# timlawrenz/DINO-X

Hardware: AMD Instinct MI355X
Metric: training images/sec (source samples; 2 global views each) ViT-S/16 224px bs256/GPU (higher is better)
Workload: dtype bf16; 1 GPU; ViT-S/16 224x224x3 2.5D slice stacks, scale-aware, 2 views/sample, DINO+Gram loss, AdamW+EMA; per_gpu_batch=256, global_batch=256, local_crops=0, out_dim=8192, parallelism=dp1, hipgraph=False

## Files before the change

### dino-x_amd/csrc/kernels.h

```cpp
#pragma once
#include <type_traits>

#include "gemm_common.h"
#include "knobs.h"

namespace dinox {

#define GEMM_VARIANTS(X)                                                                                                       \
  X(NtPp, "gemm_bf16_nt_pp") X(NtPp128, "gemm_bf16_nt_pp128") X(NtPp384, "gemm_bf16_nt_pp384") X(NtAreg, "gemm_bf16_nt_areg") \
  X(NtGlds, "gemm_bf16_nt_glds") X(Nt, "gemm_bf16_nt") X(TnBig, "gemm_bf16_tn_big") X(TnDma, "gemm_bf16_tn_dma") X(Tn, "gemm_bf16_tn")
#define X(member, name) member,
enum class GemmVariant { None, GEMM_VARIANTS(X) };
#undef X
#define X(member, name) name,
inline const char* gemm_variant_name(GemmVariant v) {
  static const char* const names[] = {nullptr, GEMM_VARIANTS(X)};
  return names[(int)v];
}
#undef X

int launch_gemm_f32(const GemmParams& p, hipStream_t st);
GemmVariant gemm_bf16_variant(const GemmParams& p);
int launch_gemm_bf16(const GemmParams& p, hipStream_t st);
int64_t gemm_bf16_ws_bytes(const GemmParams& p);
bool gemm_bf16_nt_glds_ok(const GemmParams& p);
int launch_gemm_bf16_nt_glds(const GemmParams& p, hipStream_t st);
bool gemm_bf16_nt_areg_ok(const GemmParams& p);
int launch_gemm_bf16_nt_areg(const GemmParams& p, hipStream_t st);
bool gemm_bf16_nt_pp_ok(const GemmParams& p);
int launch_gemm_bf16_nt_pp(const GemmParams& p, hipStream_t st);
bool gemm_bf16_nt_pp128_ok(const GemmParams& p);
int launch_gemm_bf16_nt_pp128(const GemmParams& p, hipStream_t st);
bool gemm_bf16_nt_pp384_ok(const GemmParams& p);
int launch_gemm_bf16_nt_pp384(const GemmParams& p, hipStream_t st);
bool gemm_bf16_nt_pp384_ln_ok(int64_t M, int K);
int launch_gemm_bf16_nt_pp384_ln(const void* a, const void* w, const float* bias, const float* residual, float* x_out, const float* gamma,
                                 const float* beta, float eps, void* y, float* mean, float* rstd, int64_t M, int K, hipStream_t st);
int pp384_lnbwd_tiles(int64_t M);
int launch_gemm_bf16_nt_pp384_lnbwd(const void* a, const void* w, const float* x, const float* gamma, const float* mean, const float* rstd,
                                    float* dx, const float* dx_add, void* dx_lowp, float* ws, int64_t M, int K, hipStream_t st);
int tn_big_plan(const GemmParams& p, int& tiles_m, int& tiles_n, int& splits, int64_t& kps);
int64_t tn_big_ws_bytes(const GemmParams& p);
int launch_gemm_bf16_tn_big(const GemmParams& p, hipStream_t st, int& splits_out, int& tiles_n_out);

int launch_attention_ref_fwd(const void* qkv, void* o, float* lse, int B, int N, int heads, int d, int dtype, hipStream_t st);
int launch_attention_ref_bwd(const void* d_o, const void* qkv, const void* o, const float* lse, void* dqkv, int B, int N, int heads, int d, int dtype, hipStream_t st);
int launch_attention_bf16_fwd(const void* qkv, void* o, float* lse, int B, int N, int heads, int d, hipStream_t st);
int launch_attention_bf16_bwd(const void* d_o, const void* qkv, const void* o, const float* lse, void* dqkv, float* ws, int B, int N, int heads, int d, hipStream_t st);
bool attention_qkv_fused_ok(int B, int N, int heads, int d, int D);
int launch_attention_qkv_fused_fwd(const void* x, const void* w, const float* bias, void* o, void* qkv_out, float* lse, int B, int N, int heads, int d, int D, hipStream_t st);
int launch_attention_flash_fwd(const void* qkv, void* o, float* lse, int B, int N, int heads, int d, hipStream_t st);
int launch_attention_flash_bwd(const void* d_o, const void* qkv, const void* o, const float* lse, void* dqkv, float* ws, int B, int N, int heads, int d, hipStream_t st);

enum { EPI_ACT_PLAIN = 0, EPI_ACT_GELU = 1, EPI_ACT_DGELU = 2 };

template <typename F>
static inline int with_epilogue_case(const GemmParams& p, F&& f) {
  const int act = (p.epilogue & DINOX_EPI_GELU) ? EPI_ACT_GELU : (p.epilogue & DINOX_EPI_DGELU) ? EPI_ACT_DGELU : EPI_ACT_PLAIN;
  const bool res = (p.epilogue & DINOX_EPI_RESIDUAL) != 0;
  auto cases = [&](auto out) -> int {
    switch (act * 2 + (res ? 1 : 0)) {
      case 0: return f(out, std::integral_constant<int, EPI_ACT_PLAIN>{}, std::false_type{});
      case 1: return f(out, std::integral_constant<int, EPI_ACT_PLAIN>{}, std::true_type{});
      case 2: return f(out, std::integral_constant<int, EPI_ACT_GELU>{}, std::false_type{});
      case 4: return f(out, std::integral_constant<int, EPI_ACT_DGELU>{}, std::false_type{});
      default: return DINOX_EUNSUPPORTED;
    }
  };
  return p.out_dtype == DINOX_BF16 ? cases(std::integral_constant<int, DINOX_BF16>{}) : cases(std::integral_constant<int, DINOX_F32>{});
}

struct PersistPlan {
  int tiles_n, units, order, stagger;
  unsigned grid;
};
static inline bool persist_plan(const GemmParams& p, int bm, int bn, int stagger_auto, PersistPlan& pl) {
  const int64_t tiles_n = ceil_div(p.N, (int64_t)bn), units = ceil_div(p.M, (int64_t)bm) * tiles_n;
  if (units > 0x3fffffff) return false;
  const int64_t ncu = device_cu_count();
  pl = {(int)tiles_n, (int)units, knob_int("DINOX_PP_ORDER", 1), knob_int("DINOX_PP_STAGGER", stagger_auto), (unsigned)(units < ncu ? units : ncu)};
  return true;
}

}
```

### dino-x_amd/csrc/loss.hip

```cpp
#include "common.h"

namespace dinox {

constexpr int CE_THREADS = 256;

__global__ __launch_bounds__(CE_THREADS) void dino_ce_kernel(const float* __restrict__ s, const float* __restrict__ t,
                                                             const float* __restrict__ center, float inv_ts, float inv_tt,
                                                             float gscale, float* __restrict__ ds,
                                                             float* __restrict__ row_loss, int rows, int K) {
  __shared__ float red[16];
  const int i = blockIdx.x, B = rows / 2;
  const int pi = (i + B) % rows;
  const float* sr = s + (int64_t)i * K;
  const float* tr = t + (int64_t)pi * K;
  float ms = -INFINITY, mt = -INFINITY;
  for (int k = threadIdx.x; k < K; k += CE_THREADS) {
    ms = fmaxf(ms, sr[k] * inv_ts);
    mt = fmaxf(mt, (tr[k] - center[k]) * inv_tt);
  }
  ms = block_max(ms, red);
  mt = block_max(mt, red);
  float ss = 0.f, st = 0.f;
  for (int k = threadIdx.x; k < K; k += CE_THREADS) {
    ss += expf(sr[k] * inv_ts - ms);
    st += expf((tr[k] - center[k]) * inv_tt - mt);
  }
  ss = block_sum(ss, red);
  st = block_sum(st, red);
  const float log_ss = logf(ss), inv_ss = 1.0f / ss, inv_st = 1.0f / st;
  float acc = 0.f;
  for (int k = threadIdx.x; k < K; k += CE_THREADS) {
    const float zs = sr[k] * inv_ts - ms;
    const float tp = expf((tr[k] - center[k]) * inv_tt - mt) * inv_st;
    acc -= tp * (zs - log_ss);
    if (ds) ds[(int64_t)i * K + k] = gscale * (expf(zs) * inv_ss - tp) * inv_ts / (float)rows;
  }
  acc = block_sum(acc, red);
  if (threadIdx.x == 0) row_loss[i] = acc;
}

__global__ __launch_bounds__(CE_THREADS) void dino_teacher_stats_kernel(const float* __restrict__ t, const float* __restrict__ center,
                                                                        float inv_tt, float* __restrict__ tmax, float* __restrict__ tinv, int K) {
  __shared__ float red[16];
  const int i = blockIdx.x;
  const float* tr = t + (int64_t)i * K;
  float m = -INFINITY;
  for (int k = threadIdx.x; k < K; k += CE_THREADS) m = fmaxf(m, (tr[k] - center[k]) * inv_tt);
  m = block_max(m, red);
  float a = 0.f;
  for (int k = threadIdx.x; k < K; k += CE_THREADS) a += expf((tr[k] - center[k]) * inv_tt - m);
  a = block_sum(a, red);
  if (threadIdx.x == 0) {
    tmax[i] = m;
// ... 188 lines not shown
}

extern "C" int dinox_colmean(const float* t, float* out, int rows, int K, void* stream) {
  DX_REQUIRE(t && out && rows > 0 && K > 0, DINOX_EINVAL, "colmean: bad arguments");
  if (K % 4 == 0 && (((uintptr_t)t | (uintptr_t)out) & 15) == 0)
    hipLaunchKernelGGL(colmean_kernel, dim3((unsigned)ceil_div(K / 4, 64)), dim3(256), 0, as_stream(stream), t, out, rows, K);
  else
    hipLaunchKernelGGL(colmean_scalar_kernel, dim3((unsigned)ceil_div(K, 256)), dim3(256), 0, as_stream(stream), t, out, rows, K);
  return check_launch("colmean");
}

extern "C" int dinox_center_ema(float* center, const float* batch_mean, float momentum, int K, void* stream) {
  DX_REQUIRE(center && batch_mean && K > 0, DINOX_EINVAL, "center_ema: bad arguments");
  hipLaunchKernelGGL(center_ema_kernel, dim3((unsigned)ceil_div(K, 256)), dim3(256), 0, as_stream(stream), center, batch_mean, momentum, K);
  return check_launch("center_ema");
}

extern "C" int dinox_gram_normalize(const float* sfeats, const float* tfeats, void* cat, void* catneg, void* shat,
                                    float* snorm, int V, int N, int D, int out_dtype, void* stream) {
  DX_REQUIRE(sfeats && tfeats && cat && catneg && shat && snorm, DINOX_EINVAL, "gram_normalize: null pointer");
  DX_REQUIRE(V > 0 && N > 1 && D > 0, DINOX_EINVAL, "gram_normalize: V=%d N=%d D=%d", V, N, D);
  DX_REQUIRE(out_dtype == DINOX_F32 || out_dtype == DINOX_BF16, DINOX_EINVAL, "gram_normalize: dtype %d", out_dtype);
  const unsigned blocks = (unsigned)ceil_div((int64_t)V * (N - 1), 4);
  if (out_dtype == DINOX_F32)
    hipLaunchKernelGGL((gram_normalize_kernel<DINOX_F32>), dim3(blocks), dim3(256), 0, as_stream(stream), sfeats, tfeats, cat, catneg, shat, snorm, V, N, D);
  else
    hipLaunchKernelGGL((gram_normalize_kernel<DINOX_BF16>), dim3(blocks), dim3(256), 0, as_stream(stream), sfeats, tfeats, cat, catneg, shat, snorm, V, N, D);
  return check_launch("gram_normalize");
}

extern "C" int dinox_sqsum(const float* x, int64_t n, float scale, float* loss, float* ws, void* stream) {
  DX_REQUIRE(x && loss && ws && n > 0, DINOX_EINVAL, "sqsum: bad arguments");
  int64_t blocks = ceil_div(n, 256 * 8);
  if (blocks > 1024) blocks = 1024;
  hipStream_t st = as_stream(stream);
  hipLaunchKernelGGL(sqsum_partial_kernel, dim3((unsigned)blocks), dim3(256), 0, st, x, n, ws);
  hipLaunchKernelGGL(final_sum_kernel, dim3(1), dim3(256), 0, st, ws, (int)blocks, scale, loss);
  return check_launch("sqsum");
}

extern "C" int dinox_gram_normalize_bwd(const float* dxh, const void* shat, const float* snorm, const float* sfeats,
                                        float* dfeats, int V, int N, int D, int shat_dtype, int accumulate, void* stream) {
  (void)sfeats;
  DX_REQUIRE(dxh && shat && snorm && dfeats, DINOX_EINVAL, "gram_normalize_bwd: null pointer");
  DX_REQUIRE(V > 0 && N > 1 && D > 0, DINOX_EINVAL, "gram_normalize_bwd: V=%d N=%d D=%d", V, N, D);
  DX_REQUIRE(shat_dtype == DINOX_F32 || shat_dtype == DINOX_BF16, DINOX_EINVAL, "gram_normalize_bwd: dtype %d", shat_dtype);
  const unsigned blocks = (unsigned)ceil_div((int64_t)V * (N - 1), 4);
  if (shat_dtype == DINOX_F32)
    hipLaunchKernelGGL((gram_normalize_bwd_kernel<DINOX_F32>), dim3(blocks), dim3(256), 0, as_stream(stream), dxh, shat, snorm, dfeats, V, N, D, accumulate);
  else
    hipLaunchKernelGGL((gram_normalize_bwd_kernel<DINOX_BF16>), dim3(blocks), dim3(256), 0, as_stream(stream), dxh, shat, snorm, dfeats, V, N, D, accumulate);
  return check_launch("gram_normalize_bwd");
}
```

### dino-x_amd/dinox/_lib.py

```python
from __future__ import annotations

import ctypes as C
import os

import torch

_HERE = os.path.dirname(os.path.abspath(__file__))
LIB_PATH = os.environ.get("DINOX_LIB") or os.path.join(_HERE, "libdinox_hip.so")

F32, BF16 = 0, 1
EPI_BIAS, EPI_GELU, EPI_DGELU, EPI_RESIDUAL, EPI_ACCUM, EPI_AUXGRAD = 1, 2, 4, 8, 16, 32

vp, i32, i64, f32 = C.c_void_p, C.c_int32, C.c_int64, C.c_float


class GemmArgs(C.Structure):
    _fields_ = [
        ("A", vp), ("B", vp), ("C", vp),
        ("M", i64), ("N", i64), ("K", i64),
        ("lda", i64), ("ldb", i64), ("ldc", i64),
        ("batch", i64), ("strideA", i64), ("strideB", i64), ("strideC", i64),
        ("transA", i32), ("transB", i32), ("in_dtype", i32), ("out_dtype", i32), ("epilogue", i32),
        ("alpha", f32),
        ("bias", vp), ("residual", vp), ("ldr", i64), ("aux", vp), ("ldaux", i64), ("colsum", vp), ("ws", vp),
# ... 9 lines not shown
        ("n1w", vp), ("n1b", vp), ("n2w", vp), ("n2b", vp), ("wqkv", vp), ("wproj", vp), ("w1", vp), ("w2", vp),
        ("bqkv", vp), ("bproj", vp), ("b1", vp), ("b2", vp),
    ]


class BlockBwdArgs(C.Structure):
    _fields_ = [
        ("V", i64), ("N", i64), ("D", i32), ("H", i32), ("heads", i32), ("reserved", i32),
        ("g", vp), ("g_lowp", vp), ("g_lowp_buf", vp),
        ("x0", vp), ("x1", vp), ("xn1", vp), ("xn2", vp), ("qkv", vp), ("o", vp), ("lse", vp), ("pre", vp), ("act", vp),
        ("mean1", vp), ("rstd1", vp), ("mean2", vp), ("rstd2", vp), ("n1w", vp), ("n2w", vp),
        ("wqkv_t", vp), ("wproj_t", vp), ("w1_t", vp), ("w2_t", vp),
        ("dwqkv", vp), ("dbqkv", vp), ("dwproj", vp), ("dbproj", vp), ("dw1", vp), ("db1", vp), ("dw2", vp), ("db2", vp),
        ("dn1w", vp), ("dn1b", vp), ("dn2w", vp), ("dn2b", vp),
        ("dpre", vp), ("dxn2", vp), ("d_o", vp), ("dqkv", vp), ("dxn1", vp), ("g1", vp), ("g1_lowp", vp), ("g0_lowp", vp),
        ("attn_ws", vp), ("ln_ws", vp), ("tn_ws", vp), ("tn_ws_bytes", i64),
    ]


SIGNATURES = {
    "dinox_version": (i32, []),
    "dinox_last_error": (C.c_char_p, []),
    "dinox_device_ok": (i32, []),
    "dinox_gemm": (i32, [C.POINTER(GemmArgs), vp]),
    "dinox_gemm_kernel_name": (C.c_char_p, [C.POINTER(GemmArgs)]),
    "dinox_gemm_ws_bytes": (i64, [C.POINTER(GemmArgs)]),
    "dinox_colsum": (i32, [vp, vp, i64, i64, i64, i32, i32, vp]),
    "dinox_linear_residual_ln_ok": (i32, [i64, i32, i32]),
    "dinox_linear_residual_ln": (i32, [vp, vp, vp, vp, vp, vp, vp, f32, vp, i32, vp, vp, i64, i32, i32, vp]),
    "dinox_layernorm_fwd": (i32, [vp, vp, vp, vp, vp, vp, i64, i32, f32, i32, vp]),
    "dinox_layernorm_bwd_ws_bytes": (i64, [i64, i32]),
    "dinox_layernorm_bwd": (i32, [vp, vp, vp, vp, vp, vp, vp, vp, vp, vp, vp, i64, i32, i32, i32, vp]),
    "dinox_linear_ln_bwd_ok": (i32, [i64, i32, i32]),
    "dinox_linear_ln_bwd": (i32, [vp, vp, vp, vp, vp, vp, vp, vp, vp, vp, vp, vp, i64, i32, i32, i32, vp]),
    "dinox_attention_fwd": (i32, [vp, vp, vp, i32, i32, i32, i32, i32, vp]),
    "dinox_attention_bwd_ws_bytes": (i64, [i32, i32, i32]),
    "dinox_attention_bwd": (i32, [vp, vp, vp, vp, vp, vp, i32, i32, i32, i32, i32, vp]),
    "dinox_qkv_attention_ok": (i32, [i32, i32, i32, i32, i32]),
    "dinox_qkv_attention_fwd": (i32, [vp, vp, vp, vp, vp, vp, i32, i32, i32, i32, i32, vp]),
    "dinox_patch_unfold": (i32, [vp, vp, i32, i32, i32, i32, i32, vp]),
    "dinox_patch_unfold_ld": (i32, [vp, vp, i32, i32, i32, i32, i32, i32, vp]),
    "dinox_tokens_fwd": (i32, [vp, vp, vp, vp, vp, vp, i32, i32, i32, i32, i32, vp]),
    "dinox_tokens_bwd": (i32, [vp, vp, vp, vp, vp, vp, i32, i32, i32, i32, i32, vp]),
    "dinox_scale_embed_fwd": (i32, [vp] * 12 + [i32, i32, i32, f32, vp]),
    "dinox_scale_embed_bwd_ws_bytes": (i64, [i32, i32, i32]),
    "dinox_scale_embed_bwd": (i32, [vp] * 17 + [i32, i32, i32, vp]),
    "dinox_dino_ce": (i32, [vp, vp, vp, f32, f32, f32, vp, vp, vp, i32, i32, vp]),
    "dinox_dino_ce_multi": (i32, [vp, vp, vp, f32, f32, f32, vp, vp, vp, i32, i32, i32, i32, vp]),
    "dinox_colmean": (i32, [vp, vp, i32, i32, vp]),
    "dinox_center_ema": (i32, [vp, vp, f32, i32, vp]),
    "dinox_gram_normalize": (i32, [vp, vp, vp, vp, vp, vp, i32, i32, i32, i32, vp]),
    "dinox_sqsum": (i32, [vp, i64, f32, vp, vp, vp]),
    "dinox_gram_normalize_bwd": (i32, [vp, vp, vp, vp, vp, i32, i32, i32, i32, i32, vp]),
    "dinox_slice_views_lds_bytes": (i64, [i32, i32]),
    "dinox_slice_views": (i32, [vp, vp, vp, vp, i32, i32, i32, vp]),
    "dinox_slice_views_patches": (i32, [vp, vp, vp, vp, i32, i32, i32, i32, i32, i32, vp]),
    "dinox_softmax_rows": (i32, [vp, vp, i64, i32, i32, i64, vp]),
    "dinox_softmax_bwd_rows": (i32, [vp, vp, vp, f32, i64, i32, i32, i64, vp]),
    "dinox_koleo_normalize": (i32, [vp, vp, vp, vp, i64, i32, f32, vp]),
    "dinox_koleo_nn": (i32, [vp, i64, vp, vp, i32, i32, i32, i32, vp, vp, vp]),
    "dinox_koleo_loss": (i32, [vp, i32, f32, vp, vp]),
    "dinox_koleo_bwd": (i32, [vp, vp, vp, vp, i32, i32, i32, i32, f32, f32, f32, vp, vp]),
    "dinox_adamw_ema": (i32, [vp, vp, vp, vp, vp, i64, f32, f32, f32, f32, f32, i32, f32, f32, vp, vp, vp]),
    "dinox_adamw_ema_dev": (i32, [vp, vp, vp, vp, vp, i64, vp, f32, f32, f32, f32, f32, f32, vp, vp, vp]),
    "dinox_sumsq": (i32, [vp, i64, vp, vp, vp]),
    "dinox_cast_bf16": (i32, [vp, vp, i64, vp]),
    "dinox_cast_transpose_bf16": (i32, [vp, vp, i32, i32, vp]),
    "dinox_cast_transpose_bf16_multi": (i32, [vp, vp, vp, i32, i64, vp]),
    "dinox_take_rows": (i32, [vp, vp, i64, i64, i32, i64, i32, vp]),
    "dinox_put_rows": (i32, [vp, vp, i64, i64, i32, i64, i32, i32, vp]),
    "dinox_axpy": (i32, [vp, vp, f32, i64, vp]),
    "dinox_lincomb3": (i32, [vp, vp, vp, f32, f32, vp, vp]),
    "dinox_zero": (i32, [vp, i64, vp]),
    "dinox_gelu_fwd": (i32, [vp, vp, i64, vp]),
    "dinox_gelu_bwd": (i32, [vp, vp, vp, i64, vp]),
    "dinox_block_forward": (i32, [C.POINTER(BlockFwdArgs), vp]),
    "dinox_block_backward": (i32, [C.POINTER(BlockBwdArgs), vp]),
    "dinox_retrieval_ws_bytes": (i64, [i64, i64, i64]),
    "dinox_retrieval_rank": (i32, [vp, i64, vp, i64, vp, i64, i64, i64, vp, vp, vp, vp, vp, vp]),
    "dinox_knn_ws_bytes": (i64, [i64, i64, i64, i32]),
    "dinox_knn_topk": (i32, [vp, i64, vp, i64, vp, i64, i64, i64, i32, vp, vp, vp, vp]),
    "dinox_gemm_timer_start": (i32, [i32]),
    "dinox_gemm_timer_stop": (i64, [C.c_char_p, i64]),
}


class DinoxLibraryError(ImportError):
    pass


def _load() -> C.CDLL:
    if not os.path.exists(LIB_PATH):
        raise DinoxLibraryError(
            f"{LIB_PATH} not found: the HIP kernel library is the only compute path of this package "
            "(no CPU/eager fallback). Build it with `python -c 'import __graft_entry__ as g; g.build()'` "
            "or `make -C dino-x_amd/csrc`.")
    try:
        lib = C.CDLL(LIB_PATH)
    except OSError as e:
        raise DinoxLibraryError(f"cannot load {LIB_PATH}: {e}") from e
    for name, (res, args) in SIGNATURES.items():
        try:
            fn = getattr(lib, name)
        except AttributeError as e:
            raise DinoxLibraryError(f"{LIB_PATH} does not export {name}; rebuild it") from e
        fn.restype = res
# ... 15 lines not shown
```

### dino-x_amd/dinox/engine.py

```python
from __future__ import annotations

import os
from dataclasses import dataclass
from typing import List, Optional, Tuple

import torch
import torch.distributed as dist

from . import ops
from .dp import GradBucketer, exchanging
from .schedule import get_lr


@dataclass
class StepHyperParams:
    lr: float = 1e-4
    min_lr: float = 1e-6
    warmup_steps: int = 2500
    max_steps: Optional[int] = None
    weight_decay: float = 0.04
    ema: float = 0.996
    teacher_temp: float = 0.04
    student_temp: float = 0.1
    center_momentum: float = 0.9
# ... 180 lines not shown
        dt = self.compute_dtype
        l0, l2 = head[0], head[2]
        pre0 = torch.empty((cls_op.shape[0], l0.weight.shape[0]), dtype=dt, device=cls_op.device) if train else None
        h0 = ops.gemm(cls_op, ops.weight_operand(l0.weight, dt), bias=l0.bias, gelu=True, aux=pre0, auxgrad=True, out_dtype=dt)
        out = ops.gemm(h0, ops.weight_operand(l2.weight, dt), bias=l2.bias, out_dtype=torch.float32)
        if train:
            ops.grad_sink.use(l0.weight, l0.bias, l2.weight, l2.bias)
        return out, (cls_op, h0, pre0)

    def _head_backward(self, head, saved, ds: torch.Tensor) -> torch.Tensor:
        dt = self.compute_dtype
        l0, l2 = head[0], head[2]
        cls_op, h0, pre0 = saved
        dy = ops.to_mode(ds, dt)
        if dt == torch.float32:
            dpre = ops.gemm(dy, l2.weight.detach(), transB=True, dgelu=True, aux=pre0, auxgrad=True, out_dtype=dt)
        else:
            dpre = ops.gemm(dy, ops.weight_operand(l2.weight, dt, transposed=True), dgelu=True, aux=pre0, auxgrad=True, out_dtype=dt)
        g2 = ops.weight_grad(dy, h0, l2.weight, l2.bias, True)
        if dt == torch.float32:
            dcls = ops.gemm(dpre, l0.weight.detach(), transB=True, out_dtype=dt)
        else:
            dcls = ops.gemm(dpre, ops.weight_operand(l0.weight, dt, transposed=True), out_dtype=dt)
        g0 = ops.weight_grad(dpre, cls_op, l0.weight, l0.bias, True)
        assert g2 == (None, None) and g0 == (None, None), "the head's parameters must live in the engine's gradient arena"
        return dcls

    def _losses_and_backward(self, s_feats, t_feats, batch, local_batch, local_spacing):
        hp, dt = self.hp, self.compute_dtype
        scale = 1.0 / self.accum
        V = s_feats.shape[0]
        with torch.no_grad():
            sf = s_feats.detach()
            t_out, _ = self._head_forward(self.teacher.head, ops.take_rows(t_feats, 0, dt), train=False)
            if local_batch is None:
                l_feats = None
                cls = ops.take_rows(sf, 0, dt)
            else:
                with torch.enable_grad():
                    l_feats = self.student.backbone(local_batch, spacing=local_spacing)
                lf = l_feats.detach()
                cls = ops.take_rows(sf, 0, dt, out_rows=V + lf.shape[0])
                ops.take_rows(lf, 0, dt, out=cls, out_row0=V)
            s_all, saved = self._head_forward(self.student.head, cls, train=True)
            if local_batch is None:
                l_dino, ds = ops.dino_ce(s_all, t_out, self.center, hp.student_temp, hp.teacher_temp, True, grad_scale=scale)
            else:
                l_dino, ds = ops.dino_ce_multi(s_all, t_out, self.center, hp.student_temp, hp.teacher_temp, 2, grad_scale=scale)
            bm = ops.colmean(t_out)
            bm_work = dist.all_reduce(bm, op=dist.ReduceOp.SUM, group=self.group, async_op=True) if exchanging(self.group) else None
            kstate = ops.koleo_begin(s_all[:V], group=self.group) if hp.koleo_weight > 0.0 else None
            dfeats = torch.empty_like(sf)
            l_gram = None
            if hp.gram_weight != 0.0:
                l_gram, gsaved = ops.gram_loss_fwd(sf, t_feats, dt)
                ops.gram_loss_bwd(gsaved, tuple(sf.shape), hp.gram_weight * scale, dfeats=dfeats, accumulate=False)
            else:
                ops.zero_(dfeats)
            l_koleo = None
            if kstate is not None:
                l_koleo, ksaved = ops.koleo_end(kstate)
                ops.axpy_(ds[:V], ops.koleo_bwd(ksaved, hp.koleo_weight * scale), 1.0)
            dcls = self._head_backward(self.student.head, saved, ds)
            ops.put_rows_(dfeats, 0, dcls)
            roots, grads = [s_feats], [dfeats]
            if l_feats is not None:
                dl = torch.empty_like(lf)
                ops.zero_(dl)
                ops.put_rows_(dl, 0, dcls, src_row0=V)
                roots.append(l_feats)
                grads.append(dl)
            loss = ops.lincomb3(l_dino, l_gram, l_koleo, hp.gram_weight, hp.koleo_weight)
        self._mark("loss")
        torch.autograd.backward(roots, grads)
        z = self._zero1
        return loss.reshape(()), l_dino.reshape(()), (l_gram if l_gram is not None else z).reshape(()), \
            (l_koleo if l_koleo is not None else z).reshape(()), bm, bm_work

    def _losses_and_backward_autograd(self, s_feats, t_feats, t_out, batch, local_batch, local_spacing):
        hp = self.hp
        if local_batch is None:
            s_out = self.student.head(s_feats[:, 0])
            l_dino = ops.DinoCEFn.apply(s_out, t_out, self.center, hp.student_temp, hp.teacher_temp)
        else:
            l_feats = self.student.backbone(local_batch, spacing=local_spacing)
            s_all = self.student.head(torch.cat([s_feats[:, 0], l_feats[:, 0]], 0))
            s_out = s_all[:s_feats.shape[0]]
            l_dino = ops.DinoCEMultiFn.apply(s_all, t_out, self.center, hp.student_temp, hp.teacher_temp, 2)
        bm = ops.colmean(t_out)
        bm_work = dist.all_reduce(bm, op=dist.ReduceOp.SUM, group=self.group, async_op=True) if exchanging(self.group) else None
        if hp.gram_weight != 0.0:
            l_gram = ops.GramLossFn.apply(s_feats, t_feats)
            loss = l_dino + hp.gram_weight * l_gram
        else:
            l_gram = torch.zeros((), device=batch.device)
            loss = l_dino
        if hp.koleo_weight > 0.0:
            l_koleo = ops.koleo_loss(s_out, group=self.group)
            loss = loss + hp.koleo_weight * l_koleo
        else:
            l_koleo = torch.zeros((), device=batch.device)
        self._mark("loss")
        (loss if self.accum == 1 else loss / self.accum).backward()
        return loss.detach(), l_dino.detach(), l_gram.detach(), l_koleo.detach(), bm, bm_work

    def scalars(self) -> dict:
        r = self.last
# ... 3 lines not shown
```

### dino-x_amd/dinox/ops.py

```python
from __future__ import annotations

import contextlib
import ctypes as C
import math
import operator
import os
import weakref
from typing import Optional

import torch

from . import _lib
from ._lib import BF16, EPI_ACCUM, EPI_AUXGRAD, EPI_BIAS, EPI_DGELU, EPI_GELU, EPI_RESIDUAL, F32, BlockBwdArgs, BlockFwdArgs, GemmArgs, check, lib

Tensor = torch.Tensor
_OVERRIDE: list = []


@contextlib.contextmanager
def compute_dtype(dtype: torch.dtype):
    if dtype not in (torch.float32, torch.bfloat16):
        raise ValueError("compute dtype must be torch.float32 or torch.bfloat16")
    _OVERRIDE.append(dtype)
    try:
# ... 1451 lines not shown
    assert src.dtype == torch.float32 and src.is_contiguous() and src.dim() == 3
    V, N, D = src.shape
    if out is None:
        out = torch.empty((out_rows or V, D), dtype=dt, device=src.device)
    check(lib.dinox_take_rows(src.data_ptr() + 4 * row * D, _p(out), V, N * D, D, out_row0, _code(dt), _stream()), "dinox_take_rows")
    return out


def put_rows_(dst: Tensor, row: int, src: Tensor, src_row0: int = 0, accumulate: bool = False) -> None:
    assert dst.dtype == torch.float32 and dst.is_contiguous() and dst.dim() == 3 and src.is_contiguous()
    V, N, D = dst.shape
    check(lib.dinox_put_rows(_p(src), dst.data_ptr() + 4 * row * D, V, N * D, D, src_row0, _code(src.dtype), int(accumulate), _stream()),
          "dinox_put_rows")


def axpy_(y: Tensor, x: Tensor, alpha: float) -> None:
    assert y.dtype == torch.float32 and x.dtype == torch.float32 and y.is_contiguous() and x.is_contiguous() and y.numel() == x.numel()
    check(lib.dinox_axpy(_p(y), _p(x), alpha, y.numel(), _stream()), "dinox_axpy")


def lincomb3(a: Tensor, b: Optional[Tensor], c: Optional[Tensor], wb: float, wc: float) -> Tensor:
    out = torch.empty(1, dtype=torch.float32, device=a.device)
    check(lib.dinox_lincomb3(_p(a), _p(b), _p(c), wb, wc, _p(out), _stream()), "dinox_lincomb3")
    return out


def zero_(t: Tensor) -> None:
    assert t.is_contiguous()
    check(lib.dinox_zero(_p(t), t.numel() * t.element_size(), _stream()), "dinox_zero")


def colmean(t: Tensor) -> Tensor:
    t = _c(t.float())
    out = torch.empty(t.shape[1], dtype=torch.float32, device=t.device)
    check(lib.dinox_colmean(_p(t), _p(out), t.shape[0], t.shape[1], _stream()), "dinox_colmean")
    return out


def center_ema_(center: Tensor, batch_mean: Tensor, momentum: float) -> None:
    assert center.is_contiguous() and center.dtype == torch.float32
    check(lib.dinox_center_ema(_p(center), _p(batch_mean), momentum, center.numel(), _stream()), "dinox_center_ema")


def gram_loss_fwd(sf: Tensor, tf: Tensor, dt: torch.dtype):
    _need_cuda(sf, tf)
    sf, tf = _c(sf.float()), _c(tf.float())
    V, N, D = sf.shape
    T = N - 1
    dev = sf.device
    cat = torch.empty((V, T, 2 * D), dtype=dt, device=dev)
    catneg = torch.empty((V, T, 2 * D), dtype=dt, device=dev)
    shat = torch.empty((V, T, D), dtype=dt, device=dev)
    snorm = torch.empty((V, T), dtype=torch.float32, device=dev)
    check(lib.dinox_gram_normalize(_p(sf), _p(tf), _p(cat), _p(catneg), _p(shat), _p(snorm), V, N, D, _code(dt), _stream()), "dinox_gram_normalize")
    diff = gemm(cat, catneg, out_dtype=torch.float32)
    loss = torch.empty(1, dtype=torch.float32, device=dev)
    ws = torch.empty(1024, dtype=torch.float32, device=dev)
    check(lib.dinox_sqsum(_p(diff), diff.numel(), 1.0 / float(V * T * T), _p(loss), _p(ws), _stream()), "dinox_sqsum")
    return loss, (diff, shat, snorm)


def gram_loss_bwd(saved, sf_shape, scale: float, dfeats: Optional[Tensor] = None, accumulate=False) -> Tensor:
    diff, shat, snorm = saved
    V, N, D = sf_shape
    T = N - 1
    dt = shat.dtype
    d_in = diff if dt == torch.float32 else cast_bf16(diff)
    dxh = gemm(d_in, shat, transA=True, transB=True, out_dtype=torch.float32, alpha=4.0 * scale / float(V * T * T))
    if dfeats is None:
        dfeats = torch.zeros((V, N, D), dtype=torch.float32, device=diff.device)
    check(lib.dinox_gram_normalize_bwd(_p(dxh), _p(shat), _p(snorm), None, _p(dfeats), V, N, D, _code(dt), int(accumulate), _stream()),
          "dinox_gram_normalize_bwd")
    return dfeats


class GramLossFn(torch.autograd.Function):

    @staticmethod
    def forward(ctx, sf, tf):
        dt = current_dtype()
        loss, saved = gram_loss_fwd(sf, tf, dt)
        ctx.save_for_backward(*saved)
        ctx.shape = tuple(sf.shape)
        return loss.reshape(())

    @staticmethod
    def backward(ctx, g):
        d = gram_loss_bwd(ctx.saved_tensors, ctx.shape, 1.0)
        return d * g, None


def koleo_begin(x: Tensor, group=None):
    import torch.distributed as dist
    _need_cuda(x)
    x = _c(x.float())
    V, D = x.shape
    dev = x.device
    from .dp import exchanging
    gather = exchanging(group)
    world = dist.get_world_size(group) if gather else 1
    rank = dist.get_rank(group) if gather else 0
    f = lambda *sh: torch.empty(sh, dtype=torch.float32, device=dev)
    xh, norm, sq = f(V, D), f(V), f(V)
    check(lib.dinox_koleo_normalize(_p(x), _p(xh), _p(norm), _p(sq), V, D, 1e-12, _stream()), "dinox_koleo_normalize")
    works = []
    if gather:
        xh_all, sq_all = f(world * V, D), f(world * V)
        works.append(dist.all_gather_into_tensor(xh_all, xh, group=group, async_op=True))
        works.append(dist.all_gather_into_tensor(sq_all, sq, group=group, async_op=True))
    else:
        xh_all, sq_all = xh, sq
    return (xh, xh_all, sq_all, norm, works, group, gather, world, rank, V, D)


def koleo_end(state, eps: float = 1e-8):
    import torch.distributed as dist
    xh, xh_all, sq_all, norm, works, group, gather, world, rank, V, D = state
    for w in works:
        w.wait()
    dev = xh.device
    f = lambda *sh: torch.empty(sh, dtype=torch.float32, device=dev)
    Vg, row0 = world * V, rank * V
    G = gemm_nt_f32_splitk(xh, xh_all)
    idx = torch.empty(V, dtype=torch.int32, device=dev)
    dmin = f(V)
    check(lib.dinox_koleo_nn(_p(G), Vg, _p(sq_all), _p(xh_all), row0, V, Vg, D, _p(idx), _p(dmin), _stream()), "dinox_koleo_nn")
# ... 186 lines not shown
```

### include/dinox.h

```cpp
#ifndef DINOX_H
#define DINOX_H

#include <stdint.h>

#ifdef __cplusplus
extern "C" {
#endif

#define DINOX_ABI_VERSION 3

#define DINOX_F32 0
#define DINOX_BF16 1

#define DINOX_OK 0
#define DINOX_EINVAL (-1)
#define DINOX_EUNSUPPORTED (-2)
#define DINOX_EALIGN (-3)

int dinox_version(void);
const char* dinox_last_error(void);
int dinox_device_ok(void);

#define DINOX_EPI_BIAS 1
#define DINOX_EPI_GELU 2
// ... 38 lines not shown
int dinox_layernorm_fwd(const float* x, const float* w, const float* b, void* y, float* mean, float* rstd,
                        int64_t rows, int dim, float eps, int out_dtype, void* stream);
int64_t dinox_layernorm_bwd_ws_bytes(int64_t rows, int dim);
int dinox_layernorm_bwd(const void* dy, const float* x, const float* w, const float* mean, const float* rstd,
                        float* dx, const float* dx_add, void* dx_lowp, float* dw, float* db, void* ws,
                        int64_t rows, int dim, int dy_dtype, int accumulate, void* stream);
int dinox_linear_ln_bwd_ok(int64_t M, int N, int K);
int dinox_linear_ln_bwd(const void* a, const void* w, const float* x, const float* gamma, const float* mean, const float* rstd,
                        float* dx, const float* dx_add, void* dx_lowp, float* dgamma, float* dbeta, void* ws, int64_t M, int N,
                        int K, int accumulate, void* stream);

int dinox_attention_fwd(const void* qkv, void* o, float* lse, int B, int N, int heads, int d, int dtype,
                        void* stream);
int dinox_softmax_rows(float* s, float* lse, int64_t rows, int n, int rows_per_image, int64_t lse_image_stride, void* stream);
int dinox_softmax_bwd_rows(float* s, float* dp, const float* lse, float scale, int64_t rows, int n, int rows_per_image,
                           int64_t lse_image_stride, void* stream);
int64_t dinox_attention_bwd_ws_bytes(int B, int N, int heads);
int dinox_attention_bwd(const void* d_o, const void* qkv, const void* o, const float* lse, void* dqkv, void* ws,
                        int B, int N, int heads, int d, int dtype, void* stream);
int dinox_qkv_attention_ok(int B, int N, int heads, int d, int D);
int dinox_qkv_attention_fwd(const void* x, const void* wqkv, const float* bias, void* o, void* qkv_out, float* lse, int B, int N,
                            int heads, int d, int D, void* stream);

int dinox_patch_unfold(const float* x, void* u, int V, int H, int W, int patch, int out_dtype, void* stream);
int dinox_patch_unfold_ld(const float* x, void* u, int V, int H, int W, int patch, int ld, int out_dtype, void* stream);
int dinox_tokens_fwd(const void* patches, const float* cls, const float* pos, const float* registers,
                     const float* scale, float* tokens, int V, int P, int R, int D, int patches_dtype,
                     void* stream);
int dinox_tokens_bwd(const float* dtokens, void* dpatches, float* dcls, float* dpos, float* dregs,
                     float* dscale, int V, int P, int R, int D, int patches_dtype, void* stream);

int dinox_scale_embed_fwd(const float* spacing, const float* w0, const float* b0, const float* w2,
                          const float* b2, const float* lnw, const float* lnb, float* out, float* hpre,
                          float* e, float* mean, float* rstd, int V, int h, int D, float eps, void* stream);
int64_t dinox_scale_embed_bwd_ws_bytes(int V, int h, int D);
int dinox_scale_embed_bwd(const float* dout, const float* spacing, const float* w0, const float* w2,
                          const float* lnw, const float* hpre, const float* e, const float* mean,
                          const float* rstd, float* dw0, float* db0, float* dw2, float* db2, float* dlnw,
                          float* dlnb, float* dspacing, void* ws, int V, int h, int D, void* stream);

int dinox_dino_ce(const float* s, const float* t, const float* center, float student_temp, float teacher_temp,
                  float grad_scale, float* loss, float* ds, float* row_loss, int rows2B, int K, void* stream);
int dinox_dino_ce_multi(const float* s, const float* t, const float* center, float student_temp, float teacher_temp,
                        float grad_scale, float* loss, float* ds, float* ws, int B, int n_global, int n_views, int K,
                        void* stream);
int dinox_colmean(const float* t, float* out, int rows, int K, void* stream);
int dinox_center_ema(float* center, const float* batch_mean, float momentum, int K, void* stream);

int dinox_gram_normalize(const float* sfeats, const float* tfeats, void* cat, void* catneg, void* shat,
                         float* snorm, int V, int N, int D, int out_dtype, void* stream);
int dinox_sqsum(const float* x, int64_t n, float scale, float* loss, float* ws, void* stream);
int dinox_gram_normalize_bwd(const float* dxh, const void* shat, const float* snorm, const float* sfeats,
                             float* dfeats, int V, int N, int D, int shat_dtype, int accumulate, void* stream);

int64_t dinox_slice_views_lds_bytes(int S, int max_crop);
int dinox_slice_views(const void* raw_u16, const int64_t* view_i, const float* view_f, float* out, int V, int S, int max_crop,
                      void* stream);
int dinox_slice_views_patches(const void* raw_u16, const int64_t* view_i, const float* view_f, void* u, int V, int S, int max_crop,
                              int patch, int ld, int out_dtype, void* stream);

int dinox_koleo_normalize(const float* x, float* xh, float* norm, float* sq, int64_t V, int D, float eps, void* stream);
int dinox_koleo_nn(const float* G, int64_t ldg, const float* sq_all, const float* xh_all, int row0, int V_l, int V_g, int D,
                   int* idx, float* dist, void* stream);
int dinox_koleo_loss(const float* dist, int V, float eps, float* loss, void* stream);
int dinox_koleo_bwd(const float* xh_all, const int* idx_all, const float* dist_all, const float* norm_loc, int row0, int V_l,
                    int V_g, int D, float gscale, float eps, float norm_eps, float* dx, void* stream);

int dinox_adamw_ema(float* p, const float* g, float* m, float* v, float* teacher, int64_t n, float lr,
                    float weight_decay, float beta1, float beta2, float eps, int step_t, float ema,
                    float grad_scale, float* gnorm_sq, float* ws, void* stream);
int dinox_adamw_ema_dev(float* p, const float* g, float* m, float* v, float* teacher, int64_t n, const float* hyper,
                        float weight_decay, float beta1, float beta2, float eps, float ema, float grad_scale,
                        float* gnorm_sq, float* ws, void* stream);
int dinox_sumsq(const float* x, int64_t n, float* out, float* ws, void* stream);
int dinox_cast_bf16(const float* src, void* dst, int64_t n, void* stream);
int dinox_cast_transpose_bf16(const float* src, void* dst, int R, int C, void* stream);
int dinox_cast_transpose_bf16_multi(const float* src_base, void* dst_base, const int64_t* table, int n_mats,
                                    int64_t total_tiles, void* stream);
int dinox_take_rows(const float* src, void* dst, int64_t V, int64_t src_stride, int D, int64_t dst_row0, int dst_dtype,
                    void* stream);
int dinox_put_rows(const void* src, float* dst, int64_t V, int64_t dst_stride, int D, int64_t src_row0, int src_dtype,
                   int accumulate, void* stream);
int dinox_axpy(float* y, const float* x, float alpha, int64_t n, void* stream);
int dinox_lincomb3(const float* a, const float* b, const float* c, float wb, float wc, float* out, void* stream);
int dinox_zero(void* p, int64_t bytes, void* stream);
int dinox_gelu_fwd(const float* x, float* y, int64_t n, void* stream);
int dinox_gelu_bwd(const float* dy, const float* x, float* dx, int64_t n, void* stream);

typedef struct dinox_block_fwd_args {
  int64_t V, N;
  int32_t D, H, heads;
  int32_t train;
  int32_t fuse_proj_ln, fuse_fc2_ln;
  float eps;
  const float* x0;
  const void* xn1_in; const float* mean1_in; const float* rstd1_in;
  void* xn1; float* mean1; float* rstd1;
  void* qkv; void* o; float* lse;
  float* x1; void* xn2; float* mean2; float* rstd2;
  void* act; void* pre;
  float* x2;
  const float* next_g; const float* next_b; float next_eps; int32_t next_dtype;
  void* yn; float* meann; float* rstdn;
  const float *n1w, *n1b, *n2w, *n2b;
  const void *wqkv, *wproj, *w1, *w2;
  const float *bqkv, *bproj, *b1, *b2;
// ... 36 lines not shown
```

Baseline: 7289 samples/s.

## Fuse Gram loss forward and backward into one per-view MFMA kernel

Adds a single kernel per view that normalizes student and teacher patch features, builds both Gram matrices with bf16 MFMA on the upper-triangle tiles, forms the difference and loss, multiplies the difference by the normalized features, and applies the normalization backward directly into dfeats. It replaces the normalize kernel, two large GEMMs, the sqsum reduction and the normalize-backward kernel, along with their intermediate buffers. The engine uses it when the shapes fit (T<=208, D<=384, D%64==0). It runs only one block per view, which may underuse the GPU, and it keeps the difference matrix in bf16.

```diff
diff --git a/dino-x_amd/csrc/gram_fused.hip b/dino-x_amd/csrc/gram_fused.hip
--- /dev/null
+++ b/dino-x_amd/csrc/gram_fused.hip
@@ -0,0 +1,296 @@
+#include "kernels.h"
+
+namespace dinox {
+
+constexpr int GF_THREADS = 512;
+constexpr int GF_TMAX = 208, GF_RT = GF_TMAX / 16;
+constexpr int GF_DMAX = 384, GF_CS = GF_DMAX / 16 / 8;
+constexpr int GF_KC = 64, GF_BSTR = GF_KC + 8;
+constexpr int GF_UP = 224, GF_DSTR = GF_UP + 8;
+constexpr int GF_UC = 32, GF_TSTR = GF_UC + 8;
+constexpr int GF_OROWS = 64, GF_OSTR = GF_DMAX + 4;
+constexpr int GF_MAXQ = 12;
+constexpr int GF_HDR = 4096;
+constexpr int GF_IMG_BYTES = GF_TMAX * GF_DSTR * 2;
+constexpr int GF_LDS_BYTES = GF_HDR + GF_IMG_BYTES + GF_DMAX * GF_TSTR * 2;
+static_assert(2 * GF_TMAX * GF_BSTR * 2 <= GF_IMG_BYTES, "pass-B staging aliases the diff image");
+static_assert(GF_OROWS * GF_OSTR * 4 <= GF_LDS_BYTES - GF_HDR, "output stage aliases image + S^ chunk");
+static_assert(3 * GF_TMAX * 4 + 64 <= GF_HDR, "norm tables");
+
+__device__ __forceinline__ uint32_t gf_pack2(float a, float b) { return (uint32_t)f32_to_bf16(a) | ((uint32_t)f32_to_bf16(b) << 16); }
+
+__global__ __launch_bounds__(GF_THREADS) void gram_loss_fused_kernel(const float* __restrict__ sf, const float* __restrict__ tf,
+                                                                     float* __restrict__ dfeats, float* __restrict__ ws, float alpha,
+                                                                     int N, int D) {
+  extern __shared__ __attribute__((aligned(16))) unsigned char gf_lds[];
+  float* inv_s = reinterpret_cast<float*>(gf_lds);
+  float* inv_t = inv_s + GF_TMAX;
+  float* nrm_s = inv_t + GF_TMAX;
+  float* red = nrm_s + GF_TMAX;
+  bf16_t* sc = reinterpret_cast<bf16_t*>(gf_lds + GF_HDR);
+  bf16_t* tc = sc + GF_TMAX * GF_BSTR;
+  bf16_t* img = reinterpret_cast<bf16_t*>(gf_lds + GF_HDR);
+  bf16_t* st = img + GF_TMAX * GF_DSTR;
+  float* stage = reinterpret_cast<float*>(gf_lds + GF_HDR);
+
+  const int tid = threadIdx.x, lane = tid & 63;
+  const int wave = __builtin_amdgcn_readfirstlane(tid >> 6);
+  const int v = blockIdx.x, T = N - 1;
+  const int nT = (T + 15) >> 4;
+  const float* sv = sf + ((int64_t)v * N + 1) * D;
+  const float* tv = tf + ((int64_t)v * N + 1) * D;
+
+  {
+    const int sub = tid & 15, nq = D >> 6;
+    for (int rb = tid >> 4; rb < GF_TMAX; rb += 64) {
+      float qs[2] = {0.f, 0.f}, qt[2] = {0.f, 0.f};
+#pragma unroll
+      for (int h = 0; h < 2; ++h) {
+        const int rc = min(rb + 32 * h, T - 1);
+        const float4* xs = reinterpret_cast<const float4*>(sv + (int64_t)rc * D);
+        const float4* xt = reinterpret_cast<const float4*>(tv + (int64_t)rc * D);
+#pragma unroll
+        for (int i = 0; i < GF_DMAX / 64; ++i)
+          if (i < nq) {
+            const float4 a = xs[sub + 16 * i], b = xt[sub + 16 * i];
+            qs[h] += (a.x * a.x + a.y * a.y) + (a.z * a.z + a.w * a.w);
+            qt[h] += (b.x * b.x + b.y * b.y) + (b.z * b.z + b.w * b.w);
+          }
+      }
+#pragma unroll
+      for (int h = 0; h < 2; ++h) {
+#pragma unroll
+        for (int o = 8; o > 0; o >>= 1) {
+          qs[h] += __shfl_xor(qs[h], o, 64);
+          qt[h] += __shfl_xor(qt[h], o, 64);
+        }
+        const int r = rb + 32 * h;
+        if (sub == 0 && r < GF_TMAX) {
+          const bool live = r < T;
+          const float ns = fmaxf(sqrtf(qs[h]), 1e-12f), nt = fmaxf(sqrtf(qt[h]), 1e-12f);
+          nrm_s[r] = live ? ns : 1.0f;
+          inv_s[r] = live ? 1.0f / ns : 0.f;
+          inv_t[r] = live ? 1.0f / nt : 0.f;
+        }
+      }
+    }
+  }
+
+  const int ntiles = nT * (nT + 1) / 2;
+  const int p0 = wave * ntiles / 8, cnt = (wave + 1) * ntiles / 8 - p0;
+  int ti[GF_MAXQ], tj[GF_MAXQ];
+  {
+    int i = 0, rem = p0;
+    while (rem >= nT - i) {
+      rem -= nT - i;
+      ++i;
+    }
+    int j = i + rem;
+#pragma unroll
+    for (int q = 0; q < GF_MAXQ; ++q) {
+      ti[q] = i;
+      tj[q] = j;
+      if (++j >= nT) {
+        ++i;
+        j = i;
+      }
+    }
+  }
+  f32x4 gs[GF_MAXQ], gt[GF_MAXQ];
+#pragma unroll
+  for (int q = 0; q < GF_MAXQ; ++q) gs[q] = gt[q] = f32x4{0.f, 0.f, 0.f, 0.f};
+
+  const int c4 = tid & 15, r0 = tid >> 4;
+  float4 ps[7], pt[7];
+  auto fetch_b = [&](int kc) {
+#pragma unroll
+    for (int it = 0; it < 7; ++it) {
+      const int r = min(r0 + 32 * it, T - 1);
+      ps[it] = *reinterpret_cast<const float4*>(sv + (int64_t)r * D + kc * GF_KC + c4 * 4);
+      pt[it] = *reinterpret_cast<const float4*>(tv + (int64_t)r * D + kc * GF_KC + c4 * 4);
+    }
+  };
+  const int nkc = D / GF_KC;
+  fetch_b(0);
+  __syncthreads();
+  for (int kc = 0; kc < nkc; ++kc) {
+    if (kc) __syncthreads();
+#pragma unroll
+    for (int it = 0; it < 7; ++it) {
+      const int r = r0 + 32 * it;
+      if (r < GF_TMAX) {
+        const float is = inv_s[r], iv = inv_t[r];
+        *reinterpret_cast<uint2*>(sc + r * GF_BSTR + c4 * 4) = make_uint2(gf_pack2(ps[it].x * is, ps[it].y * is), gf_pack2(ps[it].z * is, ps[it].w * is));
+        *reinterpret_cast<uint2*>(tc + r * GF_BSTR + c4 * 4) = make_uint2(gf_pack2(pt[it].x * iv, pt[it].y * iv), gf_pack2(pt[it].z * iv, pt[it].w * iv));
+      }
+    }
+    __syncthreads();
+    if (kc + 1 < nkc) fetch_b(kc + 1);
+#pragma unroll
+    for (int ks = 0; ks < GF_KC / 32; ++ks) {
+      const int off = (lane & 15) * GF_BSTR + ks * 32 + (lane >> 4) * 8;
+      bf16x8 as = {}, at = {};
+#pragma unroll
+      for (int q = 0; q < GF_MAXQ; ++q)
+        if (q < cnt) {
+          if (q == 0 || ti[q] != ti[q - 1]) {
+            as = *reinterpret_cast<const bf16x8*>(sc + ti[q] * 16 * GF_BSTR + off);
+            at = *reinterpret_cast<const bf16x8*>(tc + ti[q] * 16 * GF_BSTR + off);
+          }
+          const bf16x8 bs = *reinterpret_cast<const bf16x8*>(sc + tj[q] * 16 * GF_BSTR + off);
+          const bf16x8 bt = *reinterpret_cast<const bf16x8*>(tc + tj[q] * 16 * GF_BSTR + off);
+          gs[q] = __builtin_amdgcn_mfma_f32_16x16x32_bf16(as, bs, gs[q], 0, 0, 0);
+          gt[q] = __builtin_amdgcn_mfma_f32_16x16x32_bf16(at, bt, gt[q], 0, 0, 0);
+        }
+    }
+  }
+
+  __syncthreads();
+  float lsum = 0.f;
+  {
+    const int n = lane & 15, rb = (lane >> 4) * 4;
+#pragma unroll
+    for (int q = 0; q < GF_MAXQ; ++q)
+      if (q < cnt) {
+        const f32x4 d = gs[q] - gt[q];
+        const float sq = (d[0] * d[0] + d[1] * d[1]) + (d[2] * d[2] + d[3] * d[3]);
+        lsum += ti[q] == tj[q] ? sq : 2.0f * sq;
+        const int row = ti[q] * 16 + rb, col = tj[q] * 16 + n;
+#pragma unroll
+        for (int r = 0; r < 4; ++r) img[(row + r) * GF_DSTR + col] = f32_to_bf16(d[r]);
+        if (ti[q] != tj[q]) *reinterpret_cast<uint2*>(img + col * GF_DSTR + row) = make_uint2(gf_pack2(d[0], d[1]), gf_pack2(d[2], d[3]));
+      }
+  }
+  const int nuc = (nT * 16 + GF_UC - 1) / GF_UC;
+  if (nuc * GF_UC > nT * 16)
+    for (int i = tid; i < nT * 16 * 16; i += GF_THREADS) img[(i >> 4) * GF_DSTR + nT * 16 + (i & 15)] = 0;
+  lsum = wave_sum(lsum);
+  if (lane == 0) red[wave] = lsum;
+
+  const int nct = D >> 4;
+  f32x4 acc[GF_RT][GF_CS];
+#pragma unroll
+  for (int rt = 0; rt < GF_RT; ++rt)
+#pragma unroll
+    for (int s = 0; s < GF_CS; ++s) acc[rt][s] = f32x4{0.f, 0.f, 0.f, 0.f};
+  constexpr int GF_CI = GF_DMAX * (GF_UC / 2) / GF_THREADS;
+  const int nci = D * (GF_UC / 2) / GF_THREADS;
+  float pa[GF_CI], pb[GF_CI];
+  auto fetch_c = [&](int uc) {
+#pragma unroll
+    for (int k = 0; k < GF_CI; ++k)
+      if (k < nci) {
+        const int it = tid + GF_THREADS * k, d = it % D, u = uc * GF_UC + 2 * (it / D);
+        pa[k] = sv[(int64_t)min(u, T - 1) * D + d];
+        pb[k] = sv[(int64_t)min(u + 1, T - 1) * D + d];
+      }
+  };
+  fetch_c(0);
+  for (int uc = 0; uc < nuc; ++uc) {
+    __syncthreads();
+#pragma unroll
+    for (int k = 0; k < GF_CI; ++k)
+      if (k < nci) {
+        const int it = tid + GF_THREADS * k, d = it % D, up = it / D, u = uc * GF_UC + 2 * up;
+        *reinterpret_cast<uint32_t*>(st + d * GF_TSTR + 2 * up) = gf_pack2(pa[k] * (u < GF_TMAX ? inv_s[u] : 0.f), pb[k] * (u + 1 < GF_TMAX ? inv_s[u + 1] : 0.f));
+      }
+    __syncthreads();
+    if (uc + 1 < nuc) fetch_c(uc + 1);
+    const int koff = (lane >> 4) * 8;
+    bf16x8 b[GF_CS];
+#pragma unroll
+    for (int s = 0; s < GF_CS; ++s) {
+      b[s] = bf16x8{};
+      if (wave + 8 * s < nct) b[s] = *reinterpret_cast<const bf16x8*>(st + ((wave + 8 * s) * 16 + (lane & 15)) * GF_TSTR + koff);
+    }
+#pragma unroll
+    for (int rt = 0; rt < GF_RT; ++rt)
+      if (rt < nT) {
+        const bf16x8 a = *reinterpret_cast<const bf16x8*>(img + (rt * 16 + (lane & 15)) * GF_DSTR + uc * GF_UC + koff);
+#pragma unroll
+        for (int s = 0; s < GF_CS; ++s)
+          if (wave + 8 * s < nct) acc[rt][s] = __builtin_amdgcn_mfma_f32_16x16x32_bf16(a, b[s], acc[rt][s], 0, 0, 0);
+      }
+  }
+  if (tid == 0) {
+    float a = 0.f;
+    for (int w = 0; w < GF_THREADS / 64; ++w) a += red[w];
+    ws[v] = a;
+  }
+
+  const int D4 = D >> 2;
+  float* dv = dfeats + ((int64_t)v * N + 1) * D;
+#pragma unroll
+  for (int g = 0; g < (GF_TMAX + GF_OROWS - 1) / GF_OROWS; ++g) {
+    if (g * GF_OROWS >= T) break;
+    __syncthreads();
+#pragma unroll
+    for (int rt = 4 * g; rt < 4 * g + 4 && rt < GF_RT; ++rt)
+      if (rt < nT) {
+#pragma unroll
+        for (int s = 0; s < GF_CS; ++s)
+          if (wave + 8 * s < nct) {
+#pragma unroll
+            for (int r = 0; r < 4; ++r)
+              stage[((rt - 4 * g) * 16 + (lane >> 4) * 4 + r) * GF_OSTR + (wave + 8 * s) * 16 + (lane & 15)] = acc[rt][s][r] * alpha;
+          }
+      }
+    __syncthreads();
+    for (int ib = 0; ib < GF_OROWS / 8; ib += 4) {
+      const int lr0 = wave * (GF_OROWS / 8) + ib, t0 = g * GF_OROWS + lr0;
+      if (t0 >= T) break;
+      float4 xv[4][2];
+#pragma unroll
+      for (int i = 0; i < 4; ++i)
+#pragma unroll
+        for (int h = 0; h < 2; ++h)
+          xv[i][h] = *reinterpret_cast<const float4*>(sv + (int64_t)min(t0 + i, T - 1) * D + min(lane + 64 * h, D4 - 1) * 4);
+#pragma unroll
+      for (int i = 0; i < 4; ++i) {
+        const int lr = lr0 + i, t = t0 + i;
+        if (t >= T) break;
+        const float nrm = nrm_s[t], inv = inv_s[t];
+        const bool clamped = !(nrm > 1e-12f);
+        float4 gv[2], hv[2];
+        float proj = 0.f;
+#pragma unroll
+        for (int h = 0; h < 2; ++h) {
+          const int c = lane + 64 * h;
+          gv[h] = hv[h] = make_float4(0.f, 0.f, 0.f, 0.f);
+          if (c < D4) {
+            const float4 x = xv[i][h];
+            gv[h] = *reinterpret_cast<const float4*>(stage + lr * GF_OSTR + c * 4);
+            hv[h] = make_float4(bf16_to_f32(f32_to_bf16(x.x * inv)), bf16_to_f32(f32_to_bf16(x.y * inv)), bf16_to_f32(f32_to_bf16(x.z * inv)),
+                                bf16_to_f32(f32_to_bf16(x.w * inv)));
+            proj += (hv[h].x * gv[h].x + hv[h].y * gv[h].y) + (hv[h].z * gv[h].z + hv[h].w * gv[h].w);
+          }
+        }
+        proj = wave_sum(proj);
+#pragma unroll
+        for (int h = 0; h < 2; ++h) {
+          const int c = lane + 64 * h;
+          if (c < D4) {
+            float4 o;
+            if (clamped) o = make_float4(gv[h].x * 1e12f, gv[h].y * 1e12f, gv[h].z * 1e12f, gv[h].w * 1e12f);
+            else o = make_float4((gv[h].x - hv[h].x * proj) * inv, (gv[h].y - hv[h].y * proj) * inv, (gv[h].z - hv[h].z * proj) * inv,
+                                 (gv[h].w - hv[h].w * proj) * inv);
+            store_stream(reinterpret_cast<float4*>(dv + (int64_t)t * D + c * 4), o);
+          }
+        }
+      }
+    }
+  }
+}
+
+bool gram_fused_ok(int V, int N, int D) {
+  return V > 0 && N > 1 && N - 1 <= GF_TMAX && D > 0 && D <= GF_DMAX && D % GF_KC == 0 && knob_int("DINOX_GRAM_FUSED", 1) != 0;
+}
+
+int launch_gram_fused(const float* sf, const float* tf, float* dfeats, float* ws, float alpha, int V, int N, int D, hipStream_t st) {
+  int rc = reserve_lds(reinterpret_cast<const void*>(gram_loss_fused_kernel), GF_LDS_BYTES, "gram_loss_fused");
+  if (rc) return rc;
+  hipLaunchKernelGGL(gram_loss_fused_kernel, dim3((unsigned)V), dim3(GF_THREADS), GF_LDS_BYTES, st, sf, tf, dfeats, ws, alpha, N, D);
+  return check_launch("gram_loss_fused");
+}
+
+}
diff --git a/dino-x_amd/csrc/kernels.h b/dino-x_amd/csrc/kernels.h
--- a/dino-x_amd/csrc/kernels.h
+++ b/dino-x_amd/csrc/kernels.h
@@ -52,6 +52,9 @@
 int launch_attention_flash_fwd(const void* qkv, void* o, float* lse, int B, int N, int heads, int d, hipStream_t st);
 int launch_attention_flash_bwd(const void* d_o, const void* qkv, const void* o, const float* lse, void* dqkv, float* ws, int B, int N, int heads, int d, hipStream_t st);
 
+bool gram_fused_ok(int V, int N, int D);
+int launch_gram_fused(const float* sf, const float* tf, float* dfeats, float* ws, float alpha, int V, int N, int D, hipStream_t st);
+
 enum { EPI_ACT_PLAIN = 0, EPI_ACT_GELU = 1, EPI_ACT_DGELU = 2 };
 
 template <typename F>
diff --git a/dino-x_amd/csrc/loss.hip b/dino-x_amd/csrc/loss.hip
--- a/dino-x_amd/csrc/loss.hip
+++ b/dino-x_amd/csrc/loss.hip
@@ -1,4 +1,4 @@
-#include "common.h"
+#include "kernels.h"
 
 namespace dinox {
 
@@ -293,3 +293,19 @@
     hipLaunchKernelGGL((gram_normalize_bwd_kernel<DINOX_BF16>), dim3(blocks), dim3(256), 0, as_stream(stream), dxh, shat, snorm, dfeats, V, N, D, accumulate);
   return check_launch("gram_normalize_bwd");
 }
+
+extern "C" int dinox_gram_fused_ok(int V, int N, int D, int dtype) { return dtype == DINOX_BF16 && gram_fused_ok(V, N, D) ? 1 : 0; }
+
+extern "C" int dinox_gram_loss_fused(const float* sfeats, const float* tfeats, float grad_scale, float* loss, float* dfeats, float* ws,
+                                     int V, int N, int D, void* stream) {
+  DX_REQUIRE(sfeats && tfeats && loss && dfeats && ws, DINOX_EINVAL, "gram_loss_fused: null pointer");
+  DX_REQUIRE(V > 0 && N > 1 && D > 0, DINOX_EINVAL, "gram_loss_fused: V=%d N=%d D=%d", V, N, D);
+  DX_REQUIRE(N - 1 <= 208 && D <= 384 && D % 64 == 0, DINOX_EUNSUPPORTED, "gram_loss_fused: N=%d D=%d outside the fused envelope (T <= 208, D <= 384, D %% 64 == 0)", N, D);
+  DX_REQUIRE((((uintptr_t)sfeats | (uintptr_t)tfeats | (uintptr_t)dfeats) & 15) == 0, DINOX_EINVAL, "gram_loss_fused: pointers must be 16-byte aligned");
+  hipStream_t st = as_stream(stream);
+  const double T = (double)(N - 1), cnt = (double)V * T * T;
+  int rc = launch_gram_fused(sfeats, tfeats, dfeats, ws, (float)(4.0 * (double)grad_scale / cnt), V, N, D, st);
+  if (rc) return rc;
+  hipLaunchKernelGGL(final_sum_kernel, dim3(1), dim3(256), 0, st, ws, V, (float)(1.0 / cnt), loss);
+  return check_launch("gram_loss_fused_sum");
+}
diff --git a/dino-x_amd/dinox/_lib.py b/dino-x_amd/dinox/_lib.py
--- a/dino-x_amd/dinox/_lib.py
+++ b/dino-x_amd/dinox/_lib.py
@@ -85,6 +85,8 @@
     "dinox_gram_normalize": (i32, [vp, vp, vp, vp, vp, vp, i32, i32, i32, i32, vp]),
     "dinox_sqsum": (i32, [vp, i64, f32, vp, vp, vp]),
     "dinox_gram_normalize_bwd": (i32, [vp, vp, vp, vp, vp, i32, i32, i32, i32, i32, vp]),
+    "dinox_gram_fused_ok": (i32, [i32, i32, i32, i32]),
+    "dinox_gram_loss_fused": (i32, [vp, vp, f32, vp, vp, vp, i32, i32, i32, vp]),
     "dinox_slice_views_lds_bytes": (i64, [i32, i32]),
     "dinox_slice_views": (i32, [vp, vp, vp, vp, i32, i32, i32, vp]),
     "dinox_slice_views_patches": (i32, [vp, vp, vp, vp, i32, i32, i32, i32, i32, i32, vp]),
diff --git a/dino-x_amd/dinox/engine.py b/dino-x_amd/dinox/engine.py
--- a/dino-x_amd/dinox/engine.py
+++ b/dino-x_amd/dinox/engine.py
@@ -256,7 +256,10 @@
             kstate = ops.koleo_begin(s_all[:V], group=self.group) if hp.koleo_weight > 0.0 else None
             dfeats = torch.empty_like(sf)
             l_gram = None
-            if hp.gram_weight != 0.0:
+            if hp.gram_weight != 0.0 and sf.dtype == t_feats.dtype == torch.float32 and sf.is_contiguous() and t_feats.is_contiguous() \
+                    and ops.gram_fused_ok(tuple(sf.shape), dt):
+                l_gram = ops.gram_loss_fused(sf, t_feats, hp.gram_weight * scale, dfeats)
+            elif hp.gram_weight != 0.0:
                 l_gram, gsaved = ops.gram_loss_fwd(sf, t_feats, dt)
                 ops.gram_loss_bwd(gsaved, tuple(sf.shape), hp.gram_weight * scale, dfeats=dfeats, accumulate=False)
             else:
diff --git a/dino-x_amd/dinox/ops.py b/dino-x_amd/dinox/ops.py
--- a/dino-x_amd/dinox/ops.py
+++ b/dino-x_amd/dinox/ops.py
@@ -1527,6 +1527,8 @@
     catneg = torch.empty((V, T, 2 * D), dtype=dt, device=dev)
     shat = torch.empty((V, T, D), dtype=dt, device=dev)
     snorm = torch.empty((V, T), dtype=torch.float32, device=dev)
+    if TRACE_KERNELS is not None:
+        TRACE_KERNELS.extend(("gram_normalize_kernel", "sqsum_partial_kernel"))
     check(lib.dinox_gram_normalize(_p(sf), _p(tf), _p(cat), _p(catneg), _p(shat), _p(snorm), V, N, D, _code(dt), _stream()), "dinox_gram_normalize")
     diff = gemm(cat, catneg, out_dtype=torch.float32)
     loss = torch.empty(1, dtype=torch.float32, device=dev)
@@ -1544,9 +1546,29 @@
     dxh = gemm(d_in, shat, transA=True, transB=True, out_dtype=torch.float32, alpha=4.0 * scale / float(V * T * T))
     if dfeats is None:
         dfeats = torch.zeros((V, N, D), dtype=torch.float32, device=diff.device)
+    if TRACE_KERNELS is not None:
+        TRACE_KERNELS.append("gram_normalize_bwd_kernel")
     check(lib.dinox_gram_normalize_bwd(_p(dxh), _p(shat), _p(snorm), None, _p(dfeats), V, N, D, _code(dt), int(accumulate), _stream()),
           "dinox_gram_normalize_bwd")
     return dfeats
+
+
+def gram_fused_ok(shape, dt: torch.dtype) -> bool:
+    V, N, D = shape
+    return bool(lib.dinox_gram_fused_ok(V, N, D, _code(dt)))
+
+
+def gram_loss_fused(sf: Tensor, tf: Tensor, grad_scale: float, dfeats: Tensor) -> Tensor:
+    _need_cuda(sf, tf, dfeats)
+    assert sf.dtype == tf.dtype == dfeats.dtype == torch.float32 and sf.shape == tf.shape == dfeats.shape
+    assert sf.is_contiguous() and tf.is_contiguous() and dfeats.is_contiguous()
+    V, N, D = sf.shape
+    loss = torch.empty(1, dtype=torch.float32, device=sf.device)
+    ws = torch.empty(V, dtype=torch.float32, device=sf.device)
+    if TRACE_KERNELS is not None:
+        TRACE_KERNELS.append("gram_loss_fused_kernel")
+    check(lib.dinox_gram_loss_fused(_p(sf), _p(tf), grad_scale, _p(loss), _p(dfeats), _p(ws), V, N, D, _stream()), "dinox_gram_loss_fused")
+    return loss
 
 
 class GramLossFn(torch.autograd.Function):
diff --git a/include/dinox.h b/include/dinox.h
--- a/include/dinox.h
+++ b/include/dinox.h
@@ -114,6 +114,9 @@
 int dinox_sqsum(const float* x, int64_t n, float scale, float* loss, float* ws, void* stream);
 int dinox_gram_normalize_bwd(const float* dxh, const void* shat, const float* snorm, const float* sfeats,
                              float* dfeats, int V, int N, int D, int shat_dtype, int accumulate, void* stream);
+int dinox_gram_fused_ok(int V, int N, int D, int dtype);
+int dinox_gram_loss_fused(const float* sfeats, const float* tfeats, float grad_scale, float* loss, float* dfeats,
+                          float* ws, int V, int N, int D, void* stream);
 
 int64_t dinox_slice_views_lds_bytes(int S, int max_crop);
 int dinox_slice_views(const void* raw_u16, const int64_t* view_i, const float* view_f, float* out, int V, int S, int max_crop,
```

After: 7354 samples/s, median of 6. About the same (+0.9%).
